# linuxing3/weekend-raytracer-wgpu

Measured on AMD Instinct MI355X. Metric: Msamples/sec (pixels x spp) at 1920x1080, 1000 spp, higher is better.
Workload: dtype f32; 1 GPU; BASELINE configs[2]: path-traced 3-sphere scene, checker-diffuse ground + glass + metal (src/main.rs:539-541), 1920x1080, 1000 spp, 8 bounces, gradient sky, seed 0; width=1920, height=1080, spp=1000, num_bounces=8, mode=pt, partition=whole frame

## Files before the change

weekend-raytracer-wgpu_amd/csrc/mirt_api.hip:

```cpp
#include <hip/hip_runtime.h>

#include <algorithm>
#include <chrono>
#include <cmath>
#include <cstdarg>
#include <cstdio>
#include <cstdlib>
#include <cstring>
#include <new>
#include <vector>

#include "../../include/mirt.h"
#include "mirt_kernels.h"
#include "mirt_bvh.h"

namespace kx = mirt::exact_build;
namespace kf = mirt::fast_build;

namespace {

thread_local char g_err[512] = "";

int fail(int status, const char* fmt, ...)
{
// ... 209 lines not shown
    int      pool_config = -1;
    int      pool_grid = -1;
    bool     fixed_strips = false;
    uint32_t gss_min_width = 0;
    double   gss_keep = 0.0;
    int      by_pixel = -1;
    uint32_t pool_blocks_per_cu = 0;
    double   grid_cell = 0.0;
    double   grid_big = 0.0;
    int      pinhole = -1;
    int      spread_units = -1;
    int      static_units = -1;
    int      pool_min_spp = -1;
    int      stream = -1;
    int      px_groups = -1;
    int      strip_cand = -1;
    int      grid_flat_y = -1;
    bool     debug_slots = false;
    uint32_t static_block = 0;
    int      static_grid = -1;
    int      timing = -1;
    bool     ext_events = true;
};

Tuning read_tuning()
{
    Tuning t;
    if (const char* e = std::getenv("MIRT_POOL_CONFIG")) { const long v = std::strtol(e, nullptr, 10); if (v >= 0 && (uint32_t)v < kx::pool_config_count()) t.pool_config = (int)v; }
    if (const char* e = std::getenv("MIRT_POOL_GRID")) t.pool_grid = (e[0] == '0') ? 0 : 1;
    if (const char* e = std::getenv("MIRT_STRIP_MODE")) t.fixed_strips = e[0] == '1';
    if (const char* e = std::getenv("MIRT_GSS_MINW")) { const uint32_t v = (uint32_t)std::atoi(e); if (v >= 1 && v <= 16) t.gss_min_width = v; }
    if (const char* e = std::getenv("MIRT_GSS_KEEP")) { const double v = std::atof(e); if (v > 0.0 && v < 64.0) t.gss_keep = v; }
    if (const char* e = std::getenv("MIRT_BY_PIXEL")) t.by_pixel = (e[0] == '1') ? 1 : 0;
    if (const char* e = std::getenv("MIRT_POOL_BLOCKS_PER_CU")) { const uint32_t v = (uint32_t)std::atoi(e); if (v >= 1) t.pool_blocks_per_cu = v; }
    if (const char* e = std::getenv("MIRT_GRID_CELL")) { const double v = std::atof(e); if (v >= 1.0 && v <= 64.0) t.grid_cell = v; }
    if (const char* e = std::getenv("MIRT_PINHOLE")) t.pinhole = (e[0] == '0') ? 0 : 1;
    if (const char* e = std::getenv("MIRT_SPREAD_UNITS")) t.spread_units = (e[0] == '0') ? 0 : 1;
    if (const char* e = std::getenv("MIRT_STATIC_UNITS")) t.static_units = (e[0] == '1') ? 1 : 0;
    if (const char* e = std::getenv("MIRT_POOL_MIN_SPP")) { const int v = std::atoi(e); if (v >= 1) t.pool_min_spp = v; }
    if (const char* e = std::getenv("MIRT_STREAM")) t.stream = std::atoi(e) != 0 ? 1 : 0;
    if (const char* e = std::getenv("MIRT_PX_GROUPS")) { const int v = std::atoi(e); if (v >= 0 && v <= 3) t.px_groups = v; }
    if (const char* e = std::getenv("MIRT_STRIP_CAND")) t.strip_cand = (e[0] == '0') ? 0 : 1;
    if (const char* e = std::getenv("MIRT_GRID_FLAT_Y")) t.grid_flat_y = (e[0] == '0') ? 0 : 1;
    if (const char* e = std::getenv("MIRT_DEBUG_SLOTS")) t.debug_slots = e[0] == '1';
    if (const char* e = std::getenv("MIRT_STATIC_BLOCK")) { const int v = std::atoi(e); if (v == 64 || v == 128 || v == 256) t.static_block = (uint32_t)v; }
    if (const char* e = std::getenv("MIRT_STATIC_GRID")) { const int v = std::atoi(e); if (v >= 1 && v <= 64) t.static_grid = v; }
    if (const char* e = std::getenv("MIRT_TIMING")) t.timing = (e[0] == '0') ? 0 : 1;
    if (const char* e = std::getenv("MIRT_EXT_EVENTS")) t.ext_events = e[0] != '0';
    if (const char* e = std::getenv("MIRT_GRID_BIG")) { const double v = std::atof(e); if (v >= 1.0 && v <= 1024.0) t.grid_big = v; }
    return t;
}

bool camera_is_pinhole(const MirtGpuCamera& cam)
{
    if (cam.lens_radius != 0.0f) return false;
    for (int k = 0; k < 3; ++k) {
        if (!std::isfinite(cam.u[k]) || !std::isfinite(cam.v[k]) || !std::isfinite(cam.eye[k])) return false;
// ... 41 lines not shown
    bool        timing = true;
    std::vector<hipStream_t> untimed_streams;
    size_t      ev_next = 0;
    size_t      ev_in_flight = 0;
    hipStream_t zero_stream = nullptr;
    hipStream_t frame_stream_b = nullptr;
    double      ms_folded = 0.0;
    uint64_t    launches_folded = 0;
    double      last_ms = 0.0;

    bool     have_scene = false;
    uint32_t n_spheres = 0, n_mats = 0;
    uint64_t n_texels = 0;
    bool     have_sky = false;
    float    sph3[12] = {};
    bool     has_image_texture = false;
    uint32_t n_shading_routines = 0;
    uint32_t queue_routine[5] = {0, 1, 2, 3, 4};
    int      pt_scene_status = MIRT_OK;
    int      parity_scene_status = MIRT_OK;
    int      pt_materials_status = MIRT_OK;
    int      parity_materials_status = MIRT_OK;
    MirtGpuCamera         cam{};
    mirt::PreparedSphere* d_spheres = nullptr;
    MirtMaterial*         d_mats = nullptr;
    mirt::PreparedMaterial* d_pmats = nullptr;
    size_t cap_pmats = 0;
    unsigned char* d_grid = nullptr;
    size_t cap_grid = 0;
    mirt::ShadeRec* d_shade = nullptr;
// ... 409 lines not shown
            c->grid_packable = gh->dims[0] * gh->dims[1] * gh->dims[2] <= mirt::kGridMaxCells;
            c->grid_flat_y = gh->dims[1] == 1u && c->tuning.grid_flat_y != 0;
        }
        if (fits_grid) {
            if ((rc = ensure_capacity(&c->d_grid, &c->cap_grid, grid.size())) != MIRT_OK) return rc;
            HIP_TRY(hipMemcpy(c->d_grid, grid.data(), grid.size(), hipMemcpyHostToDevice));
        }
    }
    c->have_sky = s->sky != nullptr;
    if (s->sky) HIP_TRY(hipMemcpy(c->d_sky, s->sky, sizeof(MirtSkyState), hipMemcpyHostToDevice));
    c->n_spheres = s->n_spheres;
    c->n_mats = s->n_materials;
    c->n_texels = s->n_texels;
    for (uint32_t i = 0; i < 3; ++i)
        for (int k = 0; k < 4; ++k) c->sph3[4 * i + k] = (s->n_spheres == 3) ? (&prep[i].cx)[k] : 0.0f;
    c->has_image_texture = false;
    for (uint32_t i = 0; i < s->n_spheres; ++i)
        if (s->spheres[i].material_idx < s->n_materials && mat_has_image[s->spheres[i].material_idx]) c->has_image_texture = true;
    if (hbm && bvh_device) {
        const double upload_ms = std::chrono::duration<double, std::milli>(std::chrono::steady_clock::now() - t_upload).count();
        if ((rc = mirt::build_bvh_device(bvh_always, s->n_spheres, c->d_spheres, c->stream, &c->bvh_scratch, &c->d_bvh, &c->cap_bvh, &dev_bvh)) != MIRT_OK) return rc;
        adopt_device_tree(c, &dev_bvh);
        if (std::getenv("MIRT_BVH_TIMING"))
            std::fprintf(stderr, "mirt_bvh_device: n=%u always_ms=%.3f upload_ms=%.3f kernels_ms=%.3f levels=%u\n", s->n_spheres, dev_bvh.always_ms,
                         upload_ms, dev_bvh.kernels_ms, dev_bvh.levels);
    } else if (hbm) {
        const size_t nb = bvh.nodes.size() * sizeof(mirt::BvhNode), rb = bvh.recs.size() * sizeof(float), ib = bvh.ids.size() * sizeof(uint32_t);
        c->bvh_off_recs = nb;
        c->bvh_off_ids = nb + rb;
        if ((rc = ensure_capacity(&c->d_bvh, &c->cap_bvh, nb + rb + ib + 16)) != MIRT_OK) return rc;
// ... 73 lines not shown
    int rc;
    if (!c->bvh_refit.ready &&
        (rc = mirt::refit_prepare(&c->bvh_refit, t, c->bvh_on_device ? &c->bvh_levels : nullptr, c->stream, &c->bvh_scratch)) != MIRT_OK)
        return rc;
    c->have_scene = false;
    float centre[3], radius, r_max, parts[3];
    const bool timed = std::getenv("MIRT_BVH_TIMING") != nullptr;
    if ((rc = mirt::refit_bvh_device(c->bvh_refit, t, c->stream, &c->bvh_scratch, &c->bvh_stage, first, count, spheres, on_device, centre, &radius, &r_max,
                                     timed ? parts : nullptr)) != MIRT_OK)
        return rc;
    if (c->n_spheres == 3) {
        mirt::PreparedSphere prep[3];
        HIP_TRY(hipMemcpy(prep, c->d_spheres, sizeof prep, hipMemcpyDeviceToHost));
        for (uint32_t i = 0; i < 3; ++i)
            for (int k = 0; k < 4; ++k) c->sph3[4 * i + k] = (&prep[i].cx)[k];
    }
    for (int k = 0; k < 3; ++k) c->bvh_centre[k] = centre[k];
    c->bvh_radius = radius;
    c->bvh_rmax = r_max;
    ++c->bvh_refits;
    c->have_scene = true;
    if (timed)
        std::fprintf(stderr, "mirt_bvh_refit: n=%u count=%u scatter_ms=%.3f refit_ms=%.3f bounds_ms=%.3f levels=%zu\n", c->n_spheres, count, parts[0],
                     parts[1], parts[2], c->bvh_refit.level_first.empty() ? (size_t)0 : c->bvh_refit.level_first.size() - 1);
    return MIRT_OK;
}

int mirt_ctx_update_spheres(MirtContext* c, uint32_t first, uint32_t count, const MirtSphere* spheres)
{
    return update_spheres(c, first, count, spheres, false);
// ... 30 lines not shown
    c->bvh_refits = 0;
    c->bvh_levels.clear();
    c->pt_scene_status = census.bad_material_index ? MIRT_ERR_MATERIAL_INDEX : c->pt_materials_status;
    c->parity_scene_status = n > 0 ? c->parity_materials_status : MIRT_OK;
    uint32_t routine_queue[5] = {0, 1, 2, 3, 4};
    set_routines(c, census.routines_seen, routine_queue);
    c->has_image_texture = census.has_image_texture;
    if ((rc = ensure_capacity(&c->d_spheres, &c->cap_spheres, (size_t)n)) != MIRT_OK) return rc;
    float prepare_ms = 0.0f;
    if ((rc = mirt::prepare_spheres_device(d_wire, n, c->d_mats, c->n_mats, routine_queue, c->d_spheres, c->stream, timed ? &prepare_ms : nullptr)) != MIRT_OK)
        return rc;
    mirt::BvhDeviceResult dev_bvh;
    if ((rc = mirt::build_bvh_device(census.always, n, c->d_spheres, c->stream, &c->bvh_scratch, &c->d_bvh, &c->cap_bvh, &dev_bvh)) != MIRT_OK) return rc;
    c->n_spheres = n;
    for (int k = 0; k < 12; ++k) c->sph3[k] = 0.0f;
    if (n == 3) {
        mirt::PreparedSphere prep[3];
        HIP_TRY(hipMemcpy(prep, c->d_spheres, sizeof prep, hipMemcpyDeviceToHost));
        for (uint32_t i = 0; i < 3; ++i)
            for (int k = 0; k < 4; ++k) c->sph3[4 * i + k] = (&prep[i].cx)[k];
    }
    adopt_device_tree(c, &dev_bvh);
    c->have_scene = true;
    if (timed)
        std::fprintf(stderr, "mirt_set_spheres: n=%u census_ms=%.3f always_ms=%.3f prepare_ms=%.3f kernels_ms=%.3f\n", n, census.census_ms,
                     census.always_ms, prepare_ms, dev_bvh.kernels_ms);
    return MIRT_OK;
}

int mirt_ctx_set_spheres(MirtContext* c, const MirtSphere* spheres, uint32_t n_spheres) { return set_spheres(c, spheres, n_spheres, false); }

int mirt_ctx_set_spheres_device(MirtContext* c, const void* d_spheres, uint32_t n_spheres) { return set_spheres(c, d_spheres, n_spheres, true); }

int mirt_ctx_set_camera(MirtContext* c, const MirtGpuCamera* cam)
{
// ... 150 lines not shown
                         !(p->flags & MIRT_FLAG_NO_GRID);
    const size_t lds_beside = scene_lds_g + c->grid_bytes;
    const size_t lds_grid_block = (size_t)c->lds_per_block / mirt::kGridPoolBlocksPerCu;
    mirt::PoolConfig pcg = kx::pool_config_grid(lds_grid_block > lds_beside ? lds_grid_block - lds_beside : 0);
    if (count && pcg.slots != mirt::kGridPoolSlotChoices[0] && pcg.slots != mirt::kGridPoolSlotChoices[1]) pcg.slots = 0;
    const size_t lds_pool_grid_block = lds_beside + pcg.lds_bytes;
    const uint32_t pool_grid_waves_per_cu = pcg.slots ? (uint32_t)(c->lds_per_cu / lds_pool_grid_block) * (pcg.threads / 64u) : 0u;
    bool pool_grid = grid_ok && c->grid_packable && pcg.slots != 0 && tune.pool_config < 0 && p->num_bounces <= 255u &&
                     !(p->flags & MIRT_FLAG_KERNEL_STRIP) && !frame_stream &&
                     ((p->flags & MIRT_FLAG_KERNEL_POOL) ||
                      (!pool && p->spp >= mirt::kPoolMinSppGrid && c->n_shading_routines >= 1 && pool_grid_waves_per_cu >= 16));
    if (tune.pool_grid == 0) pool_grid = false;
    if (pool_grid) pool = true;
    const mirt::PoolConfig pcu = pool_grid ? pcg : pc;
    const uint32_t resident_pool_waves = pool_grid ? pool_grid_waves_per_cu : pool_waves_per_cu;

    mirt::RenderArgs a{};
    a.cam = c->cam;
    { const uint32_t flag = (pt && tune.pinhole != 0 && camera_is_pinhole(c->cam)) ? 1u : 0u; std::memcpy(&a.cam._padding5, &flag, 4); }
    a.spheres = c->d_spheres; a.mats = c->d_mats; a.pmats = c->d_pmats; a.texels = c->d_texels; a.sky = c->d_sky;
    a.out = d_out; a.counters = c->d_counters + ev * mirt::kNumCounters; a.work_counter = c->d_work_counter + ev * kDispenserWords; a.accum = d_accum;
    a.n_texels = c->n_texels; a.n_spheres = c->n_spheres; a.n_mats = c->n_mats;
    a.width = p->width; a.height = p->height; a.spp = p->spp; a.num_bounces = p->num_bounces; a.flags = p->flags;
    a.seed_mix = jenkins_hash((uint32_t)p->seed ^ jenkins_hash((uint32_t)(p->seed >> 32)));
    a.sample_begin = p->sample_begin;
    a.frame_spp = pt ? p->frame_spp : 0u;
    a.frame_begin = pt ? p->frame_begin : 0u;
    a.row_begin = p->row_begin; a.tile_rows = p->tile_rows; a.n_parts = p->n_parts; a.part = p->part;
    a.out_rows = rows;
    for (int q = 0; q < 5; ++q) a.queue_routine[q] = c->queue_routine[q];
    for (int k = 0; k < 12; ++k) a.sph3[k] = c->sph3[k];
    a.n_units = (uint32_t)((npix + mirt::kStripPixels - 1) / mirt::kStripPixels);
    for (uint32_t l = 0; l <= mirt::kStripLevels; ++l) { a.lvl_unit[l] = a.n_units; a.lvl_pix[l] = (uint32_t)npix; }
    a.lvl_unit[0] = 0;
    a.lvl_pix[0] = 0;
    if (pool) {
        const uint64_t waves = (uint64_t)c->cu_count * (resident_pool_waves < 32u ? resident_pool_waves : 32u);
        uint32_t min_width = 4;
        while (min_width < mirt::kStripPixels && (uint64_t)min_width * p->spp < 512u) min_width *= 2;
        if (tune.fixed_strips) min_width = mirt::kStripPixels;
        if (tune.gss_min_width) min_width = tune.gss_min_width;
        const double keep_factor = tune.gss_keep > 0.0 ? tune.gss_keep : 4.0;
        uint64_t pix = 0, unit = 0;
        for (uint32_t l = 0; l < mirt::kStripLevels; ++l) {
            const uint32_t width = mirt::kStripPixels >> l;
            a.lvl_unit[l] = (uint32_t)unit;
// ... 9 lines not shown
            pix += level_px;
            unit += (level_px + width - 1) / width;
        }
        a.lvl_unit[mirt::kStripLevels] = (uint32_t)unit;
        a.lvl_pix[mirt::kStripLevels] = (uint32_t)npix;
        a.n_units = (uint32_t)unit;
    }
    const bool use_grid = pool_grid || (grid_ok && !pool && scene_lds_g + c->grid_bytes + 4u * 48u <= (size_t)c->lds_per_block);
    a.grid = use_grid ? c->d_grid : nullptr;
    a.grid_bytes = use_grid ? c->grid_bytes : 0u;
    a.shade = (use_grid && c->have_shade) ? c->d_shade : nullptr;
    a.grid_pool_slots = pool_grid ? pcg.slots : 0u;
    a.strip_cand = (use_grid && tune.strip_cand != 0 && (pool_grid || p->spp >= 4u)) ? 1u : 0u;
    a.grid_flat_y = (use_grid && c->grid_flat_y) ? 1u : 0u;
    a.lds_bytes = use_grid ? (uint32_t)(scene_lds_g + a.grid_bytes + (pool ? pcu.lds_bytes : 4u * 48u)) : (uint32_t)(scene_lds + (pool ? pcu.lds_bytes : 0));
    const bool hbm = c->hbm;
    const bool hbm_bvh = hbm && pt && !(p->flags & MIRT_FLAG_NO_GRID) && (!count || (p->flags & MIRT_FLAG_COUNT_GRID));
    if (hbm) {
        a.bvh_nodes = reinterpret_cast<const float4*>(c->d_bvh);
        a.bvh_recs = reinterpret_cast<const float4*>(c->d_bvh + c->bvh_off_recs);
        a.bvh_ids = reinterpret_cast<const uint32_t*>(c->d_bvh + c->bvh_off_ids);
        a.bvh_root = c->bvh_root;
        a.bvh_n_always = c->bvh_n_always;
        for (int k = 0; k < 3; ++k) a.bvh_centre[k] = c->bvh_centre[k];
        a.bvh_radius = c->bvh_radius;
        a.bvh_rmax = c->bvh_rmax;
    }
    if (!use_grid && !c->fits_flat && !hbm)
        return fail(MIRT_ERR_SCENE_TOO_LARGE, "this scene only fits LDS in the grid build of the path-traced mode "
                    "(no parity mode, no MIRT_FLAG_COUNT_WORK / MIRT_FLAG_NO_GRID / MIRT_FLAG_KERNEL_POOL)");
// ... 465 lines not shown
```

weekend-raytracer-wgpu_amd/csrc/mirt_kernels.h:

```cpp
#pragma once

#include <hip/hip_runtime.h>
#include <stdint.h>

#include "../../include/mirt.h"

namespace mirt {

struct PreparedSphere {
    float    cx, cy, cz, rr;
    float    inv_r, radius;
    uint32_t material_idx;
    uint32_t op;
};
static_assert(sizeof(PreparedSphere) == 32, "PreparedSphere must stay 2 x 16 B for ds_read_b128");

struct PreparedMaterial {
    uint32_t id;
    float    x;
    float    inv_x;
    uint32_t flags;
    float    tex[2][4];
};
static_assert(sizeof(PreparedMaterial) == 48, "PreparedMaterial is 3 x 16 B");

struct ShadeRec {
    float a[4];
    float t0[4];
    float t1[4];
    float c[4];
};
static_assert(sizeof(ShadeRec) == 64, "ShadeRec is one 64-byte line");

struct GridHeader {
    float    org[3];
    float    cell[3];
    float    inv_cell[3];
    uint32_t dims[3];
    uint32_t n_big;
// ... 90 lines not shown
    uint32_t px_groups_log2;
    uint32_t lvl_unit[6];
    uint32_t lvl_pix[6];
    uint32_t queue_routine[5];
    uint32_t lds_bytes;
    uint32_t launch_threads;
    uint32_t stream_samples;
    float    sph3[12];
    const float4*   bvh_nodes;
    const float4*   bvh_recs;
    const uint32_t* bvh_ids;
    uint32_t        bvh_root;
    uint32_t        bvh_n_always;
    float           bvh_centre[3];
    float           bvh_radius, bvh_rmax;
};
constexpr uint32_t kBvhStackBytesPerWave = 64u * MIRT_BVH_MAX_DEPTH * 4u;

constexpr uint32_t kAssembleMaxParts = 16;
struct AssembleArgs {
    const uint32_t* parts[kAssembleMaxParts];
    uint32_t*       out;
    uint64_t        part_stride_px;
    uint32_t        width, band_rows, tile_rows, n_parts;
    uint32_t        vec4;
};

struct LaunchOn {
    hipStream_t stream = nullptr;
    hipEvent_t  begin = nullptr, end = nullptr;
// ... 39 lines not shown
```

weekend-raytracer-wgpu_amd/csrc/mirt_kernels.hip:

```cpp
#include <cstdio>
#include <mutex>

#include <hip/hip_ext.h>
#include "mirt_kernels.h"
#include "mirt_device_math.h"
#include "mirt_device_resolve.h"

namespace mirt {
namespace MIRT_KNS {


struct SceneLds {
    const float*            cam;
    const PreparedSphere*   spheres;
    const MirtMaterial*     mats;
    const PreparedMaterial* pmats;
    const float*            sky;
    unsigned char*          end;
};

template <bool PT, bool MATS_IN_LDS = true>
MIRT_DEV SceneLds stage_scene(const RenderArgs& A, unsigned char* smem, bool hosek)
{
    constexpr uint32_t kMatQuads = PT ? sizeof(PreparedMaterial) / 16 : sizeof(MirtMaterial) / 16;
// ... 26 lines not shown
    S.cam = reinterpret_cast<const float*>(smem);
    S.spheres = MATS_IN_LDS ? reinterpret_cast<const PreparedSphere*>(smem + 16 * n_cam) : A.spheres;
    S.mats = MATS_IN_LDS ? reinterpret_cast<const MirtMaterial*>(smem + 16 * (n_cam + n_sph)) : A.mats;
    S.pmats = MATS_IN_LDS ? reinterpret_cast<const PreparedMaterial*>(smem + 16 * (n_cam + n_sph)) : A.pmats;
    S.sky = hosek ? reinterpret_cast<const float*>(smem + 16 * (n_cam + n_sph + n_mat)) : nullptr;
    S.end = smem + 16 * total;
    return S;
}

MIRT_DEV const RenderArgs& per_strip_args()
{
    typedef __attribute__((address_space(4))) const RenderArgs kernarg_args;
    kernarg_args* p = (kernarg_args*)__builtin_amdgcn_kernarg_segment_ptr();
    asm volatile("" : "+s"(p));
    return *(const RenderArgs*)p;
}

MIRT_DEV size_t scene_lds_bytes_dev(uint32_t n_spheres, uint32_t n_mats, bool hosek, bool mats_in_lds = true)
{
    return sizeof(MirtGpuCamera) + (mats_in_lds ? (size_t)n_spheres * sizeof(PreparedSphere) + (size_t)n_mats * sizeof(PreparedMaterial) : 0) +
           (hosek ? sizeof(MirtSkyState) : 0);
}

MIRT_DEV uint32_t abs_row(const RenderArgs& A, uint32_t i)
{
    if (A.tile_rows == 0 || A.n_parts <= 1) return A.row_begin + i;
    const uint32_t t = A.part + (i / A.tile_rows) * A.n_parts;
    return A.row_begin + t * A.tile_rows + i % A.tile_rows;
}

// ... 445 lines not shown
MIRT_DEV CamRegs load_camera(const SceneLds& S, const RenderArgs& A, const CamHeld& H)
{
    CamRegs c;
    c.eye = mk(S.cam[0], S.cam[1], S.cam[2]);
    c.hor = H.hor; c.ver = H.ver; c.llc = H.llc;
    c.cam_u = mk(S.cam[12], S.cam[13], S.cam[14]);
    c.cam_v = mk(S.cam[16], S.cam[17], S.cam[18]);
    c.lens_radius = S.cam[19];
    c.pinhole = __builtin_amdgcn_readfirstlane(bits(S.cam[23])) != 0u;
    c.inv_w = 1.0f / (float)A.width;
    c.inv_h = 1.0f / (float)A.height;
    return c;
}

template <bool RESEED = true>
MIRT_DEV void generate_primary(const RenderArgs& A, const CamRegs& C, uint32_t x, uint32_t y, uint32_t sample,
                               Rng& rng, f3& ro, f3& rd)
{
    if constexpr (RESEED) {
        const uint32_t pixel_index = x + y * A.width;
        rng.state = jenkins_hash((pixel_index ^ jenkins_hash(sample + 1u)) ^ A.seed_mix);
    }
    const float u = ((float)x + rng.next()) * C.inv_w;
    const float v = 1.0f - ((float)y + rng.next()) * C.inv_h;
    if (C.pinhole) {
        asm volatile("; generate_primary: pinhole camera" ::);
        rng.skip();
        rng.skip();
        ro = C.eye;
    } else {
        const float lr = sqrt_unit(rng.next());
        const SinCos la = sincos_small(rng.next_scaled(kTwoPi * 0x1p-32f));
        const float lpx = C.lens_radius * (lr * la.c);
        const float lpy = C.lens_radius * (lr * la.s);
        ro = C.eye + fma3(lpy, C.cam_v, lpx * C.cam_u);
    }
    rd = fma3(v, C.ver, fma3(u, C.hor, C.llc)) - ro;
}

template <bool COUNT>
MIRT_DEV void hit_sphere(const float4 s4, uint32_t i, f3 ro, f3 rd, float a, float inv_a, bool alive, float& closest, int& best,
                         Work<COUNT>& work)
{
    const f3 oc = ro - mk(s4.x, s4.y, s4.z);
    const float b = dot(oc, rd);
    const float cq = dot(oc, oc) - s4.w;
    const float disc = fma_(b, b, -(a * cq));
    if (alive && disc > 0.0f) {
        const float sq = sqrt_(disc);
        const float t0 = (-b - sq) * inv_a;
        const float t1 = (-b + sq) * inv_a;
        if constexpr (COUNT) work.add(kCntRoots, ((t0 < closest) && (t0 > kMinT)) ? 1u : 2u);
        const float kInf = __builtin_inff();
        const float c0 = (t0 > kMinT) ? t0 : kInf;
        const float c1 = (t1 > kMinT) ? t1 : kInf;
        const float t = __builtin_fminf(c0, c1);
        const bool ok = t < closest;
        closest = ok ? t : closest;
        best = ok ? (int)i : best;
    }
}

template <bool COUNT>
MIRT_DEV int nearest_hit(const SceneLds& S, uint32_t n_spheres, f3 ro, f3 rd, bool alive, float& closest_out,
                         Work<COUNT>& work)
{
    const float a = dot(rd, rd);
    const float inv_a = rcp_(a);
    float closest = kMaxT;
    int best = -1;
    if (alive) { work.add(kCntRays); work.add(kCntTests, n_spheres); }
    const float4* sph = reinterpret_cast<const float4*>(S.spheres);
    if (n_spheres == 3u) {
        const RenderArgs& AK = per_strip_args();
        const float4 s0 = make_float4(AK.sph3[0], AK.sph3[1], AK.sph3[2], AK.sph3[3]);
        const float4 s1 = make_float4(AK.sph3[4], AK.sph3[5], AK.sph3[6], AK.sph3[7]);
        const float4 s2 = make_float4(AK.sph3[8], AK.sph3[9], AK.sph3[10], AK.sph3[11]);
        hit_sphere<COUNT>(s0, 0, ro, rd, a, inv_a, alive, closest, best, work);
        hit_sphere<COUNT>(s1, 1, ro, rd, a, inv_a, alive, closest, best, work);
        hit_sphere<COUNT>(s2, 2, ro, rd, a, inv_a, alive, closest, best, work);
        closest_out = closest;
        return best;
    }
    uint32_t i = 0;
    for (; i + 3 <= n_spheres; i += 3) {
        const float4 s0 = sph[2 * i], s1 = sph[2 * i + 2], s2 = sph[2 * i + 4];
        hit_sphere<COUNT>(s0, i, ro, rd, a, inv_a, alive, closest, best, work);
        hit_sphere<COUNT>(s1, i + 1, ro, rd, a, inv_a, alive, closest, best, work);
        hit_sphere<COUNT>(s2, i + 2, ro, rd, a, inv_a, alive, closest, best, work);
    }
    for (; i < n_spheres; ++i) hit_sphere<COUNT>(sph[2 * i], i, ro, rd, a, inv_a, alive, closest, best, work);
    closest_out = closest;
    return best;
}


MIRT_DEV float max_(float a, float b) { return (b > a) ? b : a; }

#ifndef MIRT_WALK_FRESH
#define MIRT_WALK_FRESH 3
#endif
#ifndef MIRT_WALK_RESUME
#define MIRT_WALK_RESUME 3
#endif
constexpr uint32_t kWalkCellsFresh = MIRT_WALK_FRESH, kWalkCellsResume = MIRT_WALK_RESUME;

#ifdef MIRT_DIAG_STAMPS
// ... 1544 lines not shown
```

weekend-raytracer-wgpu_amd/csrc/mirt_pool_kernel.inc:

```
template <uint32_t THREADS, uint32_t SLOTS, uint32_t MINW, bool COUNT, bool HOSEK, uint32_t NQ = 5, bool GRID = false, bool FLATY = false>
__global__ __launch_bounds__(THREADS, MINW) void MIRT_POOL_KERNEL_NAME(RenderArgs A)
{
    constexpr bool TILE = MIRT_POOL_KERNEL_TILE;
    constexpr bool FRAME = MIRT_POOL_KERNEL_FRAME;
    using Lay = WavePoolLayout<SLOTS, NQ, GRID, TILE>;
    static_assert(!(GRID && TILE), "the tile build exists for flat scenes");
    static_assert(GRID || !FLATY, "FLATY: a grid one cell high");
    constexpr uint32_t OP_GEN = NQ, OP_WALK = NQ + 1, kNumOps = Lay::kQueues;
    static_assert(NQ >= 1 && NQ < kMaxQueues, "scatter queues");
    constexpr uint32_t RING = Lay::kRing;
    static_assert(SLOTS >= 64 && SLOTS <= 256 && SLOTS % 8 == 0, "slot ids are 8 bit");
    extern __shared__ __align__(16) unsigned char smem[];
    const SceneLds S = stage_scene<true, !GRID>(A, smem, HOSEK);
    const uint32_t tid = threadIdx.x;
    const uint32_t lane = tid & 63u;
    const uint32_t wave = __builtin_amdgcn_readfirstlane(tid >> 6);
    uint32_t scene_bytes = (uint32_t)scene_lds_bytes_dev(A.n_spheres, A.n_mats, HOSEK, !GRID);
    GridLds G{};
    if constexpr (GRID) { G = stage_grid(A, smem + scene_bytes); scene_bytes += A.grid_bytes; }
    constexpr bool HOLD_CAM = !GRID && !HOSEK && !TILE && !COUNT && MINW == 6;
    CamHeld CH{};
    if constexpr (HOLD_CAM) CH = hold_camera(S);
    GridConsts GC{};
    if constexpr (GRID) GC = load_grid_consts(G);
    unsigned char* pool = smem + scene_bytes + wave * Lay::kBytes;
    uint4* const L_state = reinterpret_cast<uint4*>(pool + Lay::kOffState);
    unsigned long long* const L_acc = reinterpret_cast<unsigned long long*>(pool + Lay::kOffAcc);
    unsigned char* const L_ring = pool + Lay::kOffRing;
    unsigned short* const L_cell = reinterpret_cast<unsigned short*>(pool + Lay::kOffCell);
    unsigned short* const L_cand = reinterpret_cast<unsigned short*>(pool + Lay::kOffCand);
    uint32_t* const L_cand_n = reinterpret_cast<uint32_t*>(pool + Lay::kOffCand + 2 * kMaxCand);
    TexelTile tile{ reinterpret_cast<uint32_t*>(pool + Lay::kOffTile), reinterpret_cast<float*>(pool + Lay::kOffTile + 16), 0u, 0u, 0u, 0u, 0u, 0u };
    TexelTile* const T = TILE ? &tile : nullptr;

    Work<COUNT> work;
    work.clear();
    Stamps stamps;
    stamps.start();

    for (uint32_t strip = first_unit(); strip < A.n_units; strip = next_unit_any(A, lane)) {
        const RenderArgs& AP = per_strip_args();
        uint32_t lvl = 0;
// ... 1 lines not shown
        for (uint32_t l = 1; l < kStripLevels; ++l) lvl = (strip >= AP.lvl_unit[l]) ? l : lvl;
        uint32_t unit0 = AP.lvl_unit[0], pix0 = AP.lvl_pix[0], pix_end = AP.lvl_pix[1];
#pragma unroll
        for (uint32_t l = 1; l < kStripLevels; ++l)
            if (lvl == l) { unit0 = AP.lvl_unit[l]; pix0 = AP.lvl_pix[l]; pix_end = AP.lvl_pix[l + 1]; }
        const uint32_t width_log2 = 4u - lvl;
        const uint32_t base_pix = pix0 + ((strip - unit0) << width_log2);
        const uint32_t want_pixels = 1u << width_log2;
        const uint32_t strip_pixels = (pix_end - base_pix < want_pixels) ? (pix_end - base_pix) : want_pixels;
        const uint32_t total_items = strip_pixels * AP.spp;
        const uint32_t base_ci = base_pix / AP.width;
        const uint32_t base_x = base_pix - base_ci * AP.width;
        const bool wide = AP.width >= kStripPixels;
        const uint32_t row0 = abs_row(AP, base_ci);
        const uint32_t row1 = (base_ci + 1 < AP.out_rows) ? abs_row(AP, base_ci + 1) : row0;

        for (uint32_t s = lane; s < SLOTS; s += 64) { L_ring[OP_GEN * RING + s] = (unsigned char)s; L_state[s * 3].w = 0u; }
        if (lane < kStripPixels * 3) L_acc[lane] = 0ull;
        if constexpr (TILE) tile.reset(lane);
        if constexpr (GRID) {
            uint32_t n_cand = kNoCand;
            if (AP.strip_cand != 0u && wide && base_x + strip_pixels <= AP.width)
                n_cand = strip_candidates(AP, S, base_x, strip_pixels, row0, L_cand, lane);
            if (lane == 0) *L_cand_n = n_cand;
#define MIRT_PROBE_SITE 6
#include "mirt_pool_probes.inc"
#undef MIRT_PROBE_SITE
        }
        uint32_t tail[kNumOps];
#pragma unroll
// ... 14 lines not shown
            stamps.mark(6);
            if (!ff) {
                const uint32_t key = deepest_key<0>(tail);
                const uint32_t depth = key >> 3;
                if (depth == 0) break;
                my_k = 7u - (key & 7u);
                my_n = (depth > 64u) ? 64u : depth;
                const uint32_t my_begin = depth - my_n;
#pragma unroll
                for (uint32_t k = 0; k < kNumOps; ++k) {
                    tail[k] -= (my_k == k) ? my_n : 0u;
                }

                const bool has0 = lane < my_n;
                slot = has0 ? (uint32_t)L_ring[my_k * RING + my_begin + lane] : 0u;
                const uint4 q0 = L_state[slot * 3 + 0], q1 = L_state[slot * 3 + 1], q2 = L_state[slot * 3 + 2];
                const uint32_t fl = q0.w;
                ro = mk(from_bits(q0.x), from_bits(q0.y), from_bits(q0.z));
                rd = mk(from_bits(q1.x), from_bits(q1.y), from_bits(q1.z));
                best = has0 ? (int)(fl & 0xfffu) : 0;
                if constexpr (GRID) {
                    if (my_k == OP_WALK) {
                        best = (fl >> 25) & 1u ? best : -1;
                        walk_closest = from_bits(q2.w);
                        walk_cell = L_cell[slot];
                    }
                }
                thr = mk(from_bits(q2.x), from_bits(q2.y), from_bits(q2.z));
                rng.state = q1.w;
                pix = (fl >> 12) & 0xfu;
                bounce = (fl >> 16) & 0xffu;
                missf = (fl >> 24) & 1u;
            }
            const bool has = lane < my_n;
            bool alive = has;
            if constexpr (COUNT) { if (lane == 0) work.add(kCntWaveIters); }
#define MIRT_PROBE_SITE 4
#include "mirt_pool_probes.inc"
#undef MIRT_PROBE_SITE

            stamps.mark(0);
            if (my_k == OP_GEN) {
                if (has && missf) {
                    work.add(kCntSky);
                    const f3 c = sky_color<HOSEK>(S, rd);
                    atomicAdd(&L_acc[pix * 3 + 0], (unsigned long long)to_fixed(thr.x * c.x));
                    atomicAdd(&L_acc[pix * 3 + 1], (unsigned long long)to_fixed(thr.y * c.y));
                    atomicAdd(&L_acc[pix * 3 + 2], (unsigned long long)to_fixed(thr.z * c.z));
                }
                const uint32_t item = next_item + lane;
                next_item += my_n;
                alive = has && item < total_items;
                uint32_t sample;
                if (strip_pixels == want_pixels) { sample = item >> width_log2; pix = item & (want_pixels - 1u); }
                else { sample = item / strip_pixels; pix = item - sample * strip_pixels; }
                uint32_t x = base_x + pix, y = row0;
                if (wide) { if (x >= A.width) { x -= A.width; y = row1; } }
                else { const uint32_t pi = base_pix + pix; const uint32_t ci = pi / A.width; x = pi - ci * A.width; y = abs_row(A, ci); }
                const CamRegs C = HOLD_CAM ? load_camera(S, A, CH) : load_camera(S, A);
                generate_primary(A, C, x, y, A.sample_begin + sample, rng, ro, rd);
                thr = mk(1, 1, 1);
                bounce = 0;
            } else if (GRID && my_k == OP_WALK) {
            } else {
                const f3 hp = ro;
                f3 ndir = rd, att = mk(1, 1, 1);
                if constexpr (GRID) {
                    const float4* rec = reinterpret_cast<const float4*>(&A.shade[best]);
                    const float4 ra = rec[0], t0 = rec[1];
                    const uint32_t rid = G.ops[best];
                    const float4 c4 = G.recs[best];
                    { const Scattered sc = shade_grid_hit<COUNT>(A, rid, rec, ra, t0, mk(c4.x, c4.y, c4.z), has, rd, hp, rng, work); ndir = sc.dir; att = sc.att; }
                } else {
                const PreparedSphere sp = S.spheres[best];
                const f3 hn = sp.inv_r * (hp - mk(sp.cx, sp.cy, sp.cz));
                const PreparedMaterial* m = &S.pmats[has ? sp.material_idx : 0u];
                uint32_t routine = A.queue_routine[0];
#pragma unroll
                for (uint32_t k = 1; k < NQ; ++k) routine = (my_k == k) ? A.queue_routine[k] : routine;
                if (routine == RT_LAMBERTIAN) {
                    if (has) work.add(kCntScatter0);
                    shade_lambertian(A, m, hn, rng, ndir, att, T);
                } else if (routine == RT_METAL) {
                    if (has) work.add(kCntScatter1);
                    shade_metal(A, m, rd, hn, rng, ndir, att, T);
                } else if (routine == RT_DIELECTRIC) {
                    if (has) work.add(kCntScatter2);
                    shade_dielectric(m, rd, hn, rng, ndir, att);
                } else if (routine == RT_CHECKER) {
                    if (has) work.add(kCntScatter3);
                    shade_checkerboard(A, m, hp, hn, rng, ndir, att, T);
// ... 14 lines not shown
                ro = hp;
                rd = ndir;
                thr = thr * att;
                bounce += 1;
            }

#define MIRT_PROBE_SITE 2
#include "mirt_pool_probes.inc"
#undef MIRT_PROBE_SITE
            if (my_k == OP_GEN) stamps.mark(1); else stamps.mark(2);
            const bool resume = GRID && my_k == OP_WALK;
            const bool trace = alive && (resume || bounce < A.num_bounces);
            if constexpr (COUNT) { if (trace && !resume) work.add(kCntLaneIters); }
            float closest;
            int nb;
            bool cut = false;
            if constexpr (GRID) {
                closest = walk_closest;
                nb = best;
                uint32_t n_cand = kNoCand;
                if (my_k == OP_GEN) n_cand = __builtin_amdgcn_readfirstlane(*L_cand_n);
                if (n_cand != kNoCand) {
                    closest = kMaxT;
                    nb = -1;
                    if (trace) work.add(kCntRays);
                    const float a = dot(rd, rd);
                    const float inv_a = rcp_(a);
                    const uint4* idq = reinterpret_cast<const uint4*>(L_cand);
                    for (uint32_t j0 = 0; j0 < n_cand; j0 += 8u) {
                        const uint4 q = idq[j0 >> 3];
// ... 3 lines not shown
                            if (j0 + 4u * h >= n_cand) break;
                            const uint32_t i0 = w4[2 * h] & 0xffffu, i1 = w4[2 * h] >> 16, i2 = w4[2 * h + 1] & 0xffffu, i3 = w4[2 * h + 1] >> 16;
                            const uint32_t left = n_cand - (j0 + 4u * h);
                            const float4 r0 = G.recs[i0], r1 = G.recs[left > 1u ? i1 : 0u], r2 = G.recs[left > 2u ? i2 : 0u], r3 = G.recs[left > 3u ? i3 : 0u];
                            test_sphere<COUNT>(r0, i0, ro, rd, a, inv_a, trace, closest, nb, work);
                            if (left > 1u) test_sphere<COUNT>(r1, i1, ro, rd, a, inv_a, trace, closest, nb, work);
                            if (left > 2u) test_sphere<COUNT>(r2, i2, ro, rd, a, inv_a, trace, closest, nb, work);
                            if (left > 3u) test_sphere<COUNT>(r3, i3, ro, rd, a, inv_a, trace, closest, nb, work);
                        }
                    }
                    stamps.mark(3);
                } else {
                    grid_walk<COUNT, FLATY>(S, G, ro, rd, trace, resume, resume ? kWalkCellsResume : kWalkCellsFresh, closest, nb, walk_cell, cut, work, lane, stamps, GC);
                }
            } else {
                nb = nearest_hit<COUNT>(S, A.n_spheres, ro, rd, trace, closest, work);
                stamps.mark(5);
            }
            const bool hit = trace && !cut && nb >= 0;
            if (hit) work.add(kCntHits);
            const uint32_t miss = (trace && !cut && nb < 0) ? 1u : 0u;
#define MIRT_PROBE_SITE 5
#include "mirt_pool_probes.inc"
#undef MIRT_PROBE_SITE
            const f3 hp = cut ? ro : fma3(closest, rd, ro);
            uint32_t hit_op;
            if constexpr (GRID) hit_op = 0u;
            else hit_op = S.spheres[hit ? nb : 0].op;
            const uint32_t new_op = alive ? (cut ? OP_WALK : (hit ? hit_op : OP_GEN)) : OP_NONE;

            if constexpr (kFastForwardMin <= 64u) {
                const uint32_t k2 = __builtin_amdgcn_readfirstlane(new_op);
                if (k2 != OP_NONE && my_n >= kFastForwardMin && ballot_(has && new_op != k2) == 0ull) {
                    ff = true;
                    my_k = k2;
                    ro = hp;
                    if constexpr (GRID) { best = (k2 == OP_WALK) ? nb : (nb < 0 ? 0 : nb); walk_closest = closest; }
                    else best = nb < 0 ? 0 : nb;
                    missf = miss;
                    continue;
                }
                ff = false;
            }

            if (has) {
                const uint32_t packed = (uint32_t)(nb < 0 ? 0 : nb) | (pix << 12) | (bounce << 16) | (miss << 24) | ((nb >= 0 ? 1u : 0u) << 25);
                L_state[slot * 3 + 0] = make_uint4(bits(hp.x), bits(hp.y), bits(hp.z), packed);
                L_state[slot * 3 + 1] = make_uint4(bits(rd.x), bits(rd.y), bits(rd.z), rng.state);
                L_state[slot * 3 + 2] = make_uint4(bits(thr.x), bits(thr.y), bits(thr.z), GRID ? bits(closest) : 0u);
                if constexpr (GRID) { if (cut) L_cell[slot] = (unsigned short)walk_cell; }
            }
#define MIRT_PROBE_SITE 3
#include "mirt_pool_probes.inc"
#undef MIRT_PROBE_SITE
#pragma unroll
            for (uint32_t k = 0; k < kNumOps; ++k) {
                const unsigned long long mk_ = ballot_(new_op == k);
                const uint32_t rank = __builtin_amdgcn_mbcnt_hi((uint32_t)(mk_ >> 32), __builtin_amdgcn_mbcnt_lo((uint32_t)mk_, 0u));
                if (new_op == k) L_ring[k * RING + tail[k] + rank] = (unsigned char)slot;
                tail[k] += (uint32_t)__popcll(mk_);
            }
        }

        stamps.mark(9);
// ... 27 lines not shown
```

Baseline: 91540 Msamples/s.

## Pack per-sphere hit records in LDS, route ops via hit codes, use mul24 addressing

Adds three compile-time-gated changes to the non-grid pool kernel. It stages a 64-byte per-sphere hit record (centre, inverse radius, material) in LDS, but only when this does not reduce blocks per CU. It folds the sphere's shading op into the nearest_hit return code so the post-trace op lookup is skipped. It also uses 24-bit multiply and inline mad24 asm for slot and accumulator addressing, and precomputes row pixel offsets. The aim is fewer dependent LDS loads and cheaper integer address math per bounce, at the cost of extra LDS, inline asm, and more complex packing of the returned index.

```diff
diff --git a/weekend-raytracer-wgpu_amd/csrc/mirt_api.hip b/weekend-raytracer-wgpu_amd/csrc/mirt_api.hip
--- a/weekend-raytracer-wgpu_amd/csrc/mirt_api.hip
+++ b/weekend-raytracer-wgpu_amd/csrc/mirt_api.hip
@@ -247,6 +247,7 @@
     int      pool_min_spp = -1;
     int      stream = -1;
     int      px_groups = -1;
+    int      hit_records = -1;
     int      strip_cand = -1;
     int      grid_flat_y = -1;
     bool     debug_slots = false;
@@ -274,6 +275,7 @@
     if (const char* e = std::getenv("MIRT_STREAM")) t.stream = std::atoi(e) != 0 ? 1 : 0;
     if (const char* e = std::getenv("MIRT_PX_GROUPS")) { const int v = std::atoi(e); if (v >= 0 && v <= 3) t.px_groups = v; }
     if (const char* e = std::getenv("MIRT_STRIP_CAND")) t.strip_cand = (e[0] == '0') ? 0 : 1;
+    if (const char* e = std::getenv("MIRT_HIT_RECORDS")) t.hit_records = (e[0] == '0') ? 0 : 1;
     if (const char* e = std::getenv("MIRT_GRID_FLAT_Y")) t.grid_flat_y = (e[0] == '0') ? 0 : 1;
     if (const char* e = std::getenv("MIRT_DEBUG_SLOTS")) t.debug_slots = e[0] == '1';
     if (const char* e = std::getenv("MIRT_STATIC_BLOCK")) { const int v = std::atoi(e); if (v == 64 || v == 128 || v == 256) t.static_block = (uint32_t)v; }
@@ -345,6 +347,7 @@
     uint64_t n_texels = 0;
     bool     have_sky = false;
     float    sph3[12] = {};
+    uint32_t sph3_code[3] = {};
     bool     has_image_texture = false;
     uint32_t n_shading_routines = 0;
     uint32_t queue_routine[5] = {0, 1, 2, 3, 4};
@@ -784,6 +787,7 @@
     c->n_texels = s->n_texels;
     for (uint32_t i = 0; i < 3; ++i)
         for (int k = 0; k < 4; ++k) c->sph3[4 * i + k] = (s->n_spheres == 3) ? (&prep[i].cx)[k] : 0.0f;
+    for (uint32_t i = 0; i < 3; ++i) c->sph3_code[i] = (s->n_spheres == 3) ? (i | prep[i].op << 12) : 0u;
     c->has_image_texture = false;
     for (uint32_t i = 0; i < s->n_spheres; ++i)
         if (s->spheres[i].material_idx < s->n_materials && mat_has_image[s->spheres[i].material_idx]) c->has_image_texture = true;
@@ -887,6 +891,7 @@
         HIP_TRY(hipMemcpy(prep, c->d_spheres, sizeof prep, hipMemcpyDeviceToHost));
         for (uint32_t i = 0; i < 3; ++i)
             for (int k = 0; k < 4; ++k) c->sph3[4 * i + k] = (&prep[i].cx)[k];
+        for (uint32_t i = 0; i < 3; ++i) c->sph3_code[i] = i | prep[i].op << 12;
     }
     for (int k = 0; k < 3; ++k) c->bvh_centre[k] = centre[k];
     c->bvh_radius = radius;
@@ -947,11 +952,13 @@
     if ((rc = mirt::build_bvh_device(census.always, n, c->d_spheres, c->stream, &c->bvh_scratch, &c->d_bvh, &c->cap_bvh, &dev_bvh)) != MIRT_OK) return rc;
     c->n_spheres = n;
     for (int k = 0; k < 12; ++k) c->sph3[k] = 0.0f;
+    for (int k = 0; k < 3; ++k) c->sph3_code[k] = 0u;
     if (n == 3) {
         mirt::PreparedSphere prep[3];
         HIP_TRY(hipMemcpy(prep, c->d_spheres, sizeof prep, hipMemcpyDeviceToHost));
         for (uint32_t i = 0; i < 3; ++i)
             for (int k = 0; k < 4; ++k) c->sph3[4 * i + k] = (&prep[i].cx)[k];
+        for (uint32_t i = 0; i < 3; ++i) c->sph3_code[i] = i | prep[i].op << 12;
     }
     adopt_device_tree(c, &dev_bvh);
     c->have_scene = true;
@@ -1132,6 +1139,8 @@
     if (pool_grid) pool = true;
     const mirt::PoolConfig pcu = pool_grid ? pcg : pc;
     const uint32_t resident_pool_waves = pool_grid ? pool_grid_waves_per_cu : pool_waves_per_cu;
+    const size_t hit_rec_bytes = (pool && !pool_grid && mirt::kR10A && tune.hit_records != 0 && !(hosek && pool_cfg == mirt::kTilePoolConfig))
+                                     ? mirt::pool_hit_record_bytes(c->n_spheres, lds_pool_block, (size_t)c->lds_per_cu, (size_t)c->lds_per_block, pc.threads) : 0;
 
     mirt::RenderArgs a{};
     a.cam = c->cam;
@@ -1148,6 +1157,7 @@
     a.out_rows = rows;
     for (int q = 0; q < 5; ++q) a.queue_routine[q] = c->queue_routine[q];
     for (int k = 0; k < 12; ++k) a.sph3[k] = c->sph3[k];
+    for (int k = 0; k < 3; ++k) a.sph3_code[k] = c->sph3_code[k];
     a.n_units = (uint32_t)((npix + mirt::kStripPixels - 1) / mirt::kStripPixels);
     for (uint32_t l = 0; l <= mirt::kStripLevels; ++l) { a.lvl_unit[l] = a.n_units; a.lvl_pix[l] = (uint32_t)npix; }
     a.lvl_unit[0] = 0;
@@ -1187,6 +1197,8 @@
     a.strip_cand = (use_grid && tune.strip_cand != 0 && (pool_grid || p->spp >= 4u)) ? 1u : 0u;
     a.grid_flat_y = (use_grid && c->grid_flat_y) ? 1u : 0u;
     a.lds_bytes = use_grid ? (uint32_t)(scene_lds_g + a.grid_bytes + (pool ? pcu.lds_bytes : 4u * 48u)) : (uint32_t)(scene_lds + (pool ? pcu.lds_bytes : 0));
+    a.hit_records = (!use_grid && hit_rec_bytes != 0) ? 1u : 0u;
+    if (a.hit_records) a.lds_bytes += (uint32_t)hit_rec_bytes;
     const bool hbm = c->hbm;
     const bool hbm_bvh = hbm && pt && !(p->flags & MIRT_FLAG_NO_GRID) && (!count || (p->flags & MIRT_FLAG_COUNT_GRID));
     if (hbm) {
diff --git a/weekend-raytracer-wgpu_amd/csrc/mirt_kernels.h b/weekend-raytracer-wgpu_amd/csrc/mirt_kernels.h
--- a/weekend-raytracer-wgpu_amd/csrc/mirt_kernels.h
+++ b/weekend-raytracer-wgpu_amd/csrc/mirt_kernels.h
@@ -23,6 +23,33 @@
     float    tex[2][4];
 };
 static_assert(sizeof(PreparedMaterial) == 48, "PreparedMaterial is 3 x 16 B");
+
+struct HitRecord {
+    float            cx, cy, cz, inv_r;
+    PreparedMaterial mat;
+};
+static_assert(sizeof(HitRecord) == 64, "a hit's record is sphere << 6 away");
+
+inline size_t pool_hit_record_bytes(uint32_t n_spheres, size_t block_bytes, size_t lds_per_cu, size_t lds_per_block, uint32_t threads)
+{
+    const size_t with = block_bytes + (size_t)n_spheres * sizeof(HitRecord);
+    if (n_spheres == 0 || block_bytes == 0 || threads < 64u || with > lds_per_block) return 0;
+    const size_t by_waves = 32u / (threads / 64u);
+    const size_t blocks_now = lds_per_cu / block_bytes < by_waves ? lds_per_cu / block_bytes : by_waves;
+    const size_t blocks_with = lds_per_cu / with < by_waves ? lds_per_cu / with : by_waves;
+    return blocks_with == blocks_now ? with - block_bytes : 0;
+}
+
+#ifndef MIRT_R10_A
+#define MIRT_R10_A 1
+#endif
+#ifndef MIRT_R10_B
+#define MIRT_R10_B 1
+#endif
+#ifndef MIRT_R10_C
+#define MIRT_R10_C 1
+#endif
+constexpr bool kR10A = MIRT_R10_A != 0, kR10B = MIRT_R10_B != 0, kR10C = MIRT_R10_C != 0;
 
 struct ShadeRec {
     float a[4];
@@ -143,6 +170,8 @@
     uint32_t        bvh_n_always;
     float           bvh_centre[3];
     float           bvh_radius, bvh_rmax;
+    uint32_t        sph3_code[3];
+    uint32_t        hit_records;
 };
 constexpr uint32_t kBvhStackBytesPerWave = 64u * MIRT_BVH_MAX_DEPTH * 4u;
 
diff --git a/weekend-raytracer-wgpu_amd/csrc/mirt_kernels.hip b/weekend-raytracer-wgpu_amd/csrc/mirt_kernels.hip
--- a/weekend-raytracer-wgpu_amd/csrc/mirt_kernels.hip
+++ b/weekend-raytracer-wgpu_amd/csrc/mirt_kernels.hip
@@ -64,6 +64,15 @@
     kernarg_args* p = (kernarg_args*)__builtin_amdgcn_kernarg_segment_ptr();
     asm volatile("" : "+s"(p));
     return *(const RenderArgs*)p;
+}
+
+template <uint32_t B>
+MIRT_DEV uint32_t mad24(uint32_t a, uint32_t c)
+{
+    static_assert(B <= 64u, "inline constant");
+    uint32_t r;
+    asm("v_mad_u32_u24 %0, %1, %2, %3" : "=v"(r) : "v"(a), "n"(B), "s"(c));
+    return r;
 }
 
 MIRT_DEV size_t scene_lds_bytes_dev(uint32_t n_spheres, uint32_t n_mats, bool hosek, bool mats_in_lds = true)
@@ -539,11 +548,10 @@
 }
 
 template <bool RESEED = true>
-MIRT_DEV void generate_primary(const RenderArgs& A, const CamRegs& C, uint32_t x, uint32_t y, uint32_t sample,
-                               Rng& rng, f3& ro, f3& rd)
+MIRT_DEV void generate_primary_at(const RenderArgs& A, const CamRegs& C, uint32_t x, uint32_t y, uint32_t pixel_index, uint32_t sample,
+                                  Rng& rng, f3& ro, f3& rd)
 {
     if constexpr (RESEED) {
-        const uint32_t pixel_index = x + y * A.width;
         rng.state = jenkins_hash((pixel_index ^ jenkins_hash(sample + 1u)) ^ A.seed_mix);
     }
     const float u = ((float)x + rng.next()) * C.inv_w;
@@ -561,6 +569,13 @@
         ro = C.eye + fma3(lpy, C.cam_v, lpx * C.cam_u);
     }
     rd = fma3(v, C.ver, fma3(u, C.hor, C.llc)) - ro;
+}
+
+template <bool RESEED = true>
+MIRT_DEV void generate_primary(const RenderArgs& A, const CamRegs& C, uint32_t x, uint32_t y, uint32_t sample,
+                               Rng& rng, f3& ro, f3& rd)
+{
+    generate_primary_at<RESEED>(A, C, x, y, x + y * A.width, sample, rng, ro, rd);
 }
 
 template <bool COUNT>
@@ -586,14 +601,15 @@
     }
 }
 
-template <bool COUNT>
+constexpr uint32_t kRouteShift = 12;
+template <bool COUNT, bool ROUTED = false>
 MIRT_DEV int nearest_hit(const SceneLds& S, uint32_t n_spheres, f3 ro, f3 rd, bool alive, float& closest_out,
-                         Work<COUNT>& work)
+                         Work<COUNT>& work, int miss_code = -1)
 {
     const float a = dot(rd, rd);
     const float inv_a = rcp_(a);
     float closest = kMaxT;
-    int best = -1;
+    int best = ROUTED ? miss_code : -1;
     if (alive) { work.add(kCntRays); work.add(kCntTests, n_spheres); }
     const float4* sph = reinterpret_cast<const float4*>(S.spheres);
     if (n_spheres == 3u) {
@@ -601,12 +617,14 @@
         const float4 s0 = make_float4(AK.sph3[0], AK.sph3[1], AK.sph3[2], AK.sph3[3]);
         const float4 s1 = make_float4(AK.sph3[4], AK.sph3[5], AK.sph3[6], AK.sph3[7]);
         const float4 s2 = make_float4(AK.sph3[8], AK.sph3[9], AK.sph3[10], AK.sph3[11]);
-        hit_sphere<COUNT>(s0, 0, ro, rd, a, inv_a, alive, closest, best, work);
-        hit_sphere<COUNT>(s1, 1, ro, rd, a, inv_a, alive, closest, best, work);
-        hit_sphere<COUNT>(s2, 2, ro, rd, a, inv_a, alive, closest, best, work);
+        const uint32_t i0 = ROUTED ? AK.sph3_code[0] : 0u, i1 = ROUTED ? AK.sph3_code[1] : 1u, i2 = ROUTED ? AK.sph3_code[2] : 2u;
+        hit_sphere<COUNT>(s0, i0, ro, rd, a, inv_a, alive, closest, best, work);
+        hit_sphere<COUNT>(s1, i1, ro, rd, a, inv_a, alive, closest, best, work);
+        hit_sphere<COUNT>(s2, i2, ro, rd, a, inv_a, alive, closest, best, work);
         closest_out = closest;
         return best;
     }
+    if constexpr (ROUTED) best = -1;
     uint32_t i = 0;
     for (; i + 3 <= n_spheres; i += 3) {
         const float4 s0 = sph[2 * i], s1 = sph[2 * i + 2], s2 = sph[2 * i + 4];
@@ -616,6 +634,10 @@
     }
     for (; i < n_spheres; ++i) hit_sphere<COUNT>(sph[2 * i], i, ro, rd, a, inv_a, alive, closest, best, work);
     closest_out = closest;
+    if constexpr (ROUTED) {
+        const uint32_t op = S.spheres[best < 0 ? 0 : best].op;
+        return best >= 0 ? (int)((uint32_t)best | op << kRouteShift) : miss_code;
+    }
     return best;
 }
 
diff --git a/weekend-raytracer-wgpu_amd/csrc/mirt_pool_kernel.inc b/weekend-raytracer-wgpu_amd/csrc/mirt_pool_kernel.inc
--- a/weekend-raytracer-wgpu_amd/csrc/mirt_pool_kernel.inc
+++ b/weekend-raytracer-wgpu_amd/csrc/mirt_pool_kernel.inc
@@ -6,6 +6,8 @@
     using Lay = WavePoolLayout<SLOTS, NQ, GRID, TILE>;
     static_assert(!(GRID && TILE), "the tile build exists for flat scenes");
     static_assert(GRID || !FLATY, "FLATY: a grid one cell high");
+    constexpr bool STEP10 = !GRID && !(HOSEK && TILE);
+    constexpr bool RECORDS = STEP10 && kR10A, ROUTED = STEP10 && kR10B, MUL24 = STEP10 && kR10C;
     constexpr uint32_t OP_GEN = NQ, OP_WALK = NQ + 1, kNumOps = Lay::kQueues;
     static_assert(NQ >= 1 && NQ < kMaxQueues, "scatter queues");
     constexpr uint32_t RING = Lay::kRing;
@@ -18,6 +20,22 @@
     uint32_t scene_bytes = (uint32_t)scene_lds_bytes_dev(A.n_spheres, A.n_mats, HOSEK, !GRID);
     GridLds G{};
     if constexpr (GRID) { G = stage_grid(A, smem + scene_bytes); scene_bytes += A.grid_bytes; }
+    const uint32_t L_recs = (RECORDS && A.hit_records != 0u) ? scene_bytes : 0u;
+    if constexpr (RECORDS) {
+        if (L_recs != 0u) {
+            uint4* const recs = reinterpret_cast<uint4*>(smem + scene_bytes);
+            for (uint32_t i = tid; i < A.n_spheres; i += THREADS) {
+                const PreparedSphere sp = S.spheres[i];
+                const uint4* mat = reinterpret_cast<const uint4*>(&S.pmats[sp.material_idx < A.n_mats ? sp.material_idx : 0u]);
+                recs[4 * i + 0] = make_uint4(bits(sp.cx), bits(sp.cy), bits(sp.cz), bits(sp.inv_r));
+                recs[4 * i + 1] = mat[0];
+                recs[4 * i + 2] = mat[1];
+                recs[4 * i + 3] = mat[2];
+            }
+            __syncthreads();
+            scene_bytes += A.n_spheres * (uint32_t)sizeof(HitRecord);
+        }
+    }
     constexpr bool HOLD_CAM = !GRID && !HOSEK && !TILE && !COUNT && MINW == 6;
     CamHeld CH{};
     if constexpr (HOLD_CAM) CH = hold_camera(S);
@@ -26,6 +44,12 @@
     unsigned char* pool = smem + scene_bytes + wave * Lay::kBytes;
     uint4* const L_state = reinterpret_cast<uint4*>(pool + Lay::kOffState);
     unsigned long long* const L_acc = reinterpret_cast<unsigned long long*>(pool + Lay::kOffAcc);
+    const auto state_of = [&](uint32_t s) { return MUL24 ? reinterpret_cast<uint4*>(pool + Lay::kOffState + __umul24(s, 48u)) : L_state + s * 3; };
+    typedef __attribute__((address_space(3))) unsigned char lds_byte;
+    const auto state_of_stored = [&](uint32_t s) {
+        return MUL24 ? (uint4*)(unsigned char*)(lds_byte*)(uintptr_t)mad24<48u>(s, (uint32_t)(uintptr_t)(lds_byte*)pool + Lay::kOffState) : L_state + s * 3;
+    };
+    const auto acc_of = [&](uint32_t p) { return MUL24 ? reinterpret_cast<unsigned long long*>(pool + Lay::kOffAcc + __umul24(p, 24u)) : L_acc + p * 3; };
     unsigned char* const L_ring = pool + Lay::kOffRing;
     unsigned short* const L_cell = reinterpret_cast<unsigned short*>(pool + Lay::kOffCell);
     unsigned short* const L_cand = reinterpret_cast<unsigned short*>(pool + Lay::kOffCand);
@@ -57,6 +81,7 @@
         const bool wide = AP.width >= kStripPixels;
         const uint32_t row0 = abs_row(AP, base_ci);
         const uint32_t row1 = (base_ci + 1 < AP.out_rows) ? abs_row(AP, base_ci + 1) : row0;
+        const uint32_t row0_px = row0 * AP.width, row1_px = row1 * AP.width;
 
         for (uint32_t s = lane; s < SLOTS; s += 64) { L_ring[OP_GEN * RING + s] = (unsigned char)s; L_state[s * 3].w = 0u; }
         if (lane < kStripPixels * 3) L_acc[lane] = 0ull;
@@ -101,7 +126,8 @@
 
                 const bool has0 = lane < my_n;
                 slot = has0 ? (uint32_t)L_ring[my_k * RING + my_begin + lane] : 0u;
-                const uint4 q0 = L_state[slot * 3 + 0], q1 = L_state[slot * 3 + 1], q2 = L_state[slot * 3 + 2];
+                const uint4* const st = state_of(slot);
+                const uint4 q0 = st[0], q1 = st[1], q2 = st[2];
                 const uint32_t fl = q0.w;
                 ro = mk(from_bits(q0.x), from_bits(q0.y), from_bits(q0.z));
                 rd = mk(from_bits(q1.x), from_bits(q1.y), from_bits(q1.z));
@@ -131,9 +157,10 @@
                 if (has && missf) {
                     work.add(kCntSky);
                     const f3 c = sky_color<HOSEK>(S, rd);
-                    atomicAdd(&L_acc[pix * 3 + 0], (unsigned long long)to_fixed(thr.x * c.x));
-                    atomicAdd(&L_acc[pix * 3 + 1], (unsigned long long)to_fixed(thr.y * c.y));
-                    atomicAdd(&L_acc[pix * 3 + 2], (unsigned long long)to_fixed(thr.z * c.z));
+                    unsigned long long* const sums = acc_of(pix);
+                    atomicAdd(&sums[0], (unsigned long long)to_fixed(thr.x * c.x));
+                    atomicAdd(&sums[1], (unsigned long long)to_fixed(thr.y * c.y));
+                    atomicAdd(&sums[2], (unsigned long long)to_fixed(thr.z * c.z));
                 }
                 const uint32_t item = next_item + lane;
                 next_item += my_n;
@@ -141,11 +168,12 @@
                 uint32_t sample;
                 if (strip_pixels == want_pixels) { sample = item >> width_log2; pix = item & (want_pixels - 1u); }
                 else { sample = item / strip_pixels; pix = item - sample * strip_pixels; }
-                uint32_t x = base_x + pix, y = row0;
-                if (wide) { if (x >= A.width) { x -= A.width; y = row1; } }
-                else { const uint32_t pi = base_pix + pix; const uint32_t ci = pi / A.width; x = pi - ci * A.width; y = abs_row(A, ci); }
+                uint32_t x = base_x + pix, y = row0, row_px = row0_px;
+                if (wide) { if (x >= A.width) { x -= A.width; y = row1; row_px = row1_px; } }
+                else { const uint32_t pi = base_pix + pix; const uint32_t ci = pi / A.width; x = pi - ci * A.width; y = abs_row(A, ci); row_px = y * A.width; }
                 const CamRegs C = HOLD_CAM ? load_camera(S, A, CH) : load_camera(S, A);
-                generate_primary(A, C, x, y, A.sample_begin + sample, rng, ro, rd);
+                if constexpr (MUL24) generate_primary_at(A, C, x, y, x + row_px, A.sample_begin + sample, rng, ro, rd);
+                else generate_primary(A, C, x, y, A.sample_begin + sample, rng, ro, rd);
                 thr = mk(1, 1, 1);
                 bounce = 0;
             } else if (GRID && my_k == OP_WALK) {
@@ -159,9 +187,19 @@
                     const float4 c4 = G.recs[best];
                     { const Scattered sc = shade_grid_hit<COUNT>(A, rid, rec, ra, t0, mk(c4.x, c4.y, c4.z), has, rd, hp, rng, work); ndir = sc.dir; att = sc.att; }
                 } else {
-                const PreparedSphere sp = S.spheres[best];
-                const f3 hn = sp.inv_r * (hp - mk(sp.cx, sp.cy, sp.cz));
-                const PreparedMaterial* m = &S.pmats[has ? sp.material_idx : 0u];
+                float4 cr;
+                const PreparedMaterial* m;
+                if (L_recs != 0u) {
+                    const unsigned char* const rec = smem + (L_recs + ((uint32_t)best << 6));
+                    cr = *reinterpret_cast<const float4*>(rec);
+                    m = reinterpret_cast<const PreparedMaterial*>(rec + 16);
+                } else {
+                    const PreparedSphere sp = S.spheres[best];
+                    cr = make_float4(sp.cx, sp.cy, sp.cz, sp.inv_r);
+                    const uint32_t mi = has ? sp.material_idx : 0u;
+                    m = MUL24 ? reinterpret_cast<const PreparedMaterial*>(reinterpret_cast<const unsigned char*>(S.pmats) + __umul24(mi, 48u)) : &S.pmats[mi];
+                }
+                const f3 hn = cr.w * (hp - mk(cr.x, cr.y, cr.z));
                 uint32_t routine = A.queue_routine[0];
 #pragma unroll
                 for (uint32_t k = 1; k < NQ; ++k) routine = (my_k == k) ? A.queue_routine[k] : routine;
@@ -206,6 +244,7 @@
             if constexpr (COUNT) { if (trace && !resume) work.add(kCntLaneIters); }
             float closest;
             int nb;
+            uint32_t routed_op = 0u;
             bool cut = false;
             if constexpr (GRID) {
                 closest = walk_closest;
@@ -239,10 +278,16 @@
                     grid_walk<COUNT, FLATY>(S, G, ro, rd, trace, resume, resume ? kWalkCellsResume : kWalkCellsFresh, closest, nb, walk_cell, cut, work, lane, stamps, GC);
                 }
             } else {
+                if constexpr (ROUTED) {
+                    const int code = nearest_hit<COUNT, true>(S, A.n_spheres, ro, rd, trace, closest, work, (int)(0x80000000u | OP_GEN << kRouteShift));
+                    routed_op = ((uint32_t)code >> kRouteShift) & 7u;
+                    nb = code;
+                } else
                 nb = nearest_hit<COUNT>(S, A.n_spheres, ro, rd, trace, closest, work);
                 stamps.mark(5);
             }
             const bool hit = trace && !cut && nb >= 0;
+            const uint32_t nb_idx = ROUTED ? (uint32_t)nb & ((1u << kRouteShift) - 1u) : (uint32_t)(nb < 0 ? 0 : nb);
             if (hit) work.add(kCntHits);
             const uint32_t miss = (trace && !cut && nb < 0) ? 1u : 0u;
 #define MIRT_PROBE_SITE 5
@@ -251,8 +296,9 @@
             const f3 hp = cut ? ro : fma3(closest, rd, ro);
             uint32_t hit_op;
             if constexpr (GRID) hit_op = 0u;
+            else if constexpr (ROUTED) hit_op = routed_op;
             else hit_op = S.spheres[hit ? nb : 0].op;
-            const uint32_t new_op = alive ? (cut ? OP_WALK : (hit ? hit_op : OP_GEN)) : OP_NONE;
+            const uint32_t new_op = ROUTED ? (alive ? hit_op : OP_NONE) : alive ? (cut ? OP_WALK : (hit ? hit_op : OP_GEN)) : OP_NONE;
 
             if constexpr (kFastForwardMin <= 64u) {
                 const uint32_t k2 = __builtin_amdgcn_readfirstlane(new_op);
@@ -261,7 +307,7 @@
                     my_k = k2;
                     ro = hp;
                     if constexpr (GRID) { best = (k2 == OP_WALK) ? nb : (nb < 0 ? 0 : nb); walk_closest = closest; }
-                    else best = nb < 0 ? 0 : nb;
+                    else best = (int)nb_idx;
                     missf = miss;
                     continue;
                 }
@@ -269,10 +315,11 @@
             }
 
             if (has) {
-                const uint32_t packed = (uint32_t)(nb < 0 ? 0 : nb) | (pix << 12) | (bounce << 16) | (miss << 24) | ((nb >= 0 ? 1u : 0u) << 25);
-                L_state[slot * 3 + 0] = make_uint4(bits(hp.x), bits(hp.y), bits(hp.z), packed);
-                L_state[slot * 3 + 1] = make_uint4(bits(rd.x), bits(rd.y), bits(rd.z), rng.state);
-                L_state[slot * 3 + 2] = make_uint4(bits(thr.x), bits(thr.y), bits(thr.z), GRID ? bits(closest) : 0u);
+                const uint32_t packed = nb_idx | (pix << 12) | (bounce << 16) | (miss << 24) | ((nb >= 0 ? 1u : 0u) << 25);
+                uint4* const st = state_of_stored(slot);
+                st[0] = make_uint4(bits(hp.x), bits(hp.y), bits(hp.z), packed);
+                st[1] = make_uint4(bits(rd.x), bits(rd.y), bits(rd.z), rng.state);
+                st[2] = make_uint4(bits(thr.x), bits(thr.y), bits(thr.z), GRID ? bits(closest) : 0u);
                 if constexpr (GRID) { if (cut) L_cell[slot] = (unsigned short)walk_cell; }
             }
 #define MIRT_PROBE_SITE 3
```

After: 91460 Msamples/s. About the same (-0.1%).
